# openai/robogym

Measured on AMD Instinct MI355X. Metric: env-steps/sec (whole node) dactyl/locked batch 8192; qpos L∞ vs MuJoCo (as restated by the in-repo CPU oracle: parity unpinned), higher is better.
Workload: dtype f32

## Files before the change

include/rgstep.h:

```cpp
#ifndef RGSTEP_H
#define RGSTEP_H
#include <stddef.h>
#include <stdint.h>

#ifdef __cplusplus
extern "C" {
#endif

typedef struct rg_model rg_model;
typedef struct rg_batch rg_batch;

enum {
  RG_F_QPOS = 0,
  RG_F_QVEL = 1,
  RG_F_CTRL = 2,
  RG_F_PID = 3,
  RG_F_WARMSTART = 4,
  RG_F_TIME = 5,
  RG_F_STATUS = 6,
  RG_F_STATS = 7,
  RG_F_DEBUG = 8,
  RG_F_COST = 9,
  RG_F_PAIRLB = 10,
  RG_F_ENVPRM = 11
// ... 108 lines not shown
  const float *u, *n, *e;
  const long long* action_index;
  const float* bins; int nbins;
  float* action_out;
  const float* qpos; int qpos_stride;
  const int* hand_q;
  const float* pos_to_ctrl;
  float* prm; int prm_stride;
  int p_ctrlrange, p_timestep, p_xfrc_cube, p_mass_cube;
  int relative_action, nsubsteps, fixed_wrist, wrist_act, wrist_qadr;
  float wrist_lo, wrist_hi;
  const float* obs; int obs_stride;
  const float *goal_pos, *goal_quat, *qpos_goal;
  const int* is_goal_achieved;
  const float* contact; int contact_stride, ncon_slots;
  const float* ncon; int ncon_stride;
  const float* env_reward;
  const unsigned char* env_done;
  const int* successes_so_far;
  float *out, *reward_out;
  unsigned char *done_out, *fell_out;
  int* info_out;
  float occ_geom[5]; int n_occ;
  float timestep0, cube_body_z, fall_z, occ_cutoff, ff_p, cf_p, freeze_scale, drop_reward, clip;
  int min_episode_length;
  float unc[4];
} rg_wrap_args;
int rg_wrap_layout(const rg_wrap_dims* dims, rg_wrap_lay* lay);
int rg_wrap_pre_step(const rg_wrap_args* args, void* stream);
int rg_wrap_post_step(const rg_wrap_args* args, void* stream);
int rg_wrap_args_size(void);
int rg_batch_set_constants(rg_batch* b, const int* mask_dev, void* stream);
int rg_batch_mpr_pair(rg_batch* b, int g1, int g2, float margin, float* out_dev, void* stream);
int rg_batch_items_info(const rg_batch* b, int* slots, int* queues);
int rg_obs_dim(const rg_batch* b);
int rg_debug_size(void);
int rg_lds_bytes(void);
int rg_lds_bytes_cfg(int config);
typedef struct rb_model rb_model;
typedef struct rb_batch rb_batch;
rb_model* rb_model_create(const void* blob, size_t nbytes, char* err, int errlen);
rb_model* rb_compile_mjcf(const char* xml, const char* meshdir, char* err, int errlen);
int rb_model_enable_env_params(rb_model* m);
int rb_prm_layout(const rb_model* m, int* out, int n);
int rb_model_blob_keys(const rb_model* m, char* out, int outlen);
void rb_model_free(rb_model* m);
int rb_model_info(const rb_model* m, int* out, int n);
int rb_scratch_offset(const rb_model* m, int which);
rb_batch* rb_batch_create(const rb_model* m, int B);
void rb_batch_free(rb_batch* b);
int rb_batch_reset(rb_batch* b);
int rb_batch_set_env(rb_batch* b, int hand_qposadr, int n_hand_jnt, int relative_action, const float* pos_to_ctrl);
int rb_batch_set_action_limits(rb_batch* b, float max_position_change, unsigned ctrl_centre_mask);
void* rb_batch_field_ptr(rb_batch* b, int field, int* row_words);
int rb_batch_step(rb_batch* b, const float* action_dev, const int* active_dev, int nsubsteps, int nforward_ticks, int flags, void* stream);
int rb_batch_step_ex(rb_batch* b, const float* action_dev, const int* active_dev, const int* hold_dev, const int* nticks_dev, int nsubsteps, int nforward_ticks, int flags, void* stream);
enum {
  RB_F_MOCAP = 12,
  RB_F_EQ_DATA = 13,
  RB_F_EQ_ACTIVE = 14,
  RB_F_SENSORDATA = 15
};
typedef struct rb_tcp_args {
  int arm_qposadr[6], main_arm_qposadr[6];
  int main_gripper_actuator, tcp_body, wrist_joint, reset_controller_error;
  float max_position_change, speed_roll, speed_pitch, joint_drift_threshold, gripper_ctrl_lo, gripper_ctrl_hi;
// ... 119 lines not shown
```

robogym_amd/_native.py:

```python
import ctypes
import os

import numpy as np

_HERE = os.path.dirname(os.path.abspath(__file__))
LIB_PATH = os.environ.get("RGSTEP_LIB") or os.path.join(_HERE, "csrc", "librgstep.so")

RG_F_QPOS, RG_F_QVEL, RG_F_CTRL, RG_F_PID, RG_F_WARMSTART, RG_F_TIME, RG_F_STATUS, RG_F_STATS, RG_F_DEBUG, RG_F_COST, RG_F_PAIRLB, RG_F_ENVPRM = range(12)
RB_F_MOCAP, RB_F_EQ_DATA, RB_F_EQ_ACTIVE, RB_F_SENSORDATA = 12, 13, 14, 15
RG_STATUS_BAD_STATE, RG_STATUS_CON_FULL, RG_STATUS_CAND_FULL, RG_STATUS_ROW_FULL, RG_STATUS_BAD_FACTOR, RG_STATUS_BAD_ACTION = 1, 2, 4, 8, 16, 32


class StepArgs(ctypes.Structure):

    _fields_ = [("action_dev", ctypes.c_void_p), ("goal_quat_dev", ctypes.c_void_p), ("obs_dev", ctypes.c_void_p), ("goal_dist_dev", ctypes.c_void_p),
                ("active_dev", ctypes.c_void_p), ("hold_dev", ctypes.c_void_p), ("nticks_dev", ctypes.c_void_p), ("order_dev", ctypes.c_void_p),
                ("nsubsteps", ctypes.c_int), ("nforward_ticks", ctypes.c_int), ("flags", ctypes.c_int), ("stream", ctypes.c_void_p),
                ("config", ctypes.c_int), ("redo_dev", ctypes.c_void_p), ("preticks_dev", ctypes.c_void_p), ("xdata_dev", ctypes.c_void_p)]


RG_CFG_ROLLOUT, RG_CFG_LARGE = 0, 1
RG_POST_NDRAW = 2 + 4 + 3 + 20


# ... 97 lines not shown

    _fields_ = [(n, ctypes.c_int) for n in ("nq", "nv", "nu", "nh", "ntip", "ndelta", "randomize", "relative_goal")]


class WrapLay(ctypes.Structure):

    _fields_ = ([(n, ctypes.c_int) for n in ("fwidth", "iwidth", "W", "s_prev", "s_ema", "s_alpha", "s_aema", "s_hist", "s_slack", "s_cdown", "s_cup", "s_anmult", "s_anadd", "s_addb",
                                             "s_mulb", "s_ts", "s_wind", "s_occl", "s_ffbuf", "s_ffleft", "s_cfleft", "s_cfbuf", "s_delta", "i_emat", "i_steps", "i_drops", "i_first",
                                             "i_delay", "n_action", "n_wind")]
                + [("n_noise", ctypes.c_int * 4)] + [(n, ctypes.c_int) for n in ("u_ts", "u_wind", "u_axis", "u_ff", "u_cf")] + [("key", ctypes.c_int * len(RG_WRAP_KEYS))])


def _wrap_fields():
    p_, i_, f_ = ctypes.c_void_p, ctypes.c_int, ctypes.c_float
    return ([("B", i_), ("device", i_), ("dims", WrapDims), ("lay", WrapLay), ("fstate", p_), ("istate", p_), ("u", p_), ("n", p_), ("e", p_),
             ("action_index", p_), ("bins", p_), ("nbins", i_), ("action_out", p_), ("qpos", p_), ("qpos_stride", i_), ("hand_q", p_), ("pos_to_ctrl", p_),
             ("prm", p_), ("prm_stride", i_)]
            + [(n, i_) for n in ("p_ctrlrange", "p_timestep", "p_xfrc_cube", "p_mass_cube", "relative_action", "nsubsteps", "fixed_wrist", "wrist_act", "wrist_qadr")]
            + [("wrist_lo", f_), ("wrist_hi", f_), ("obs", p_), ("obs_stride", i_), ("goal_pos", p_), ("goal_quat", p_), ("qpos_goal", p_), ("is_goal_achieved", p_),
               ("contact", p_), ("contact_stride", i_), ("ncon_slots", i_), ("ncon", p_), ("ncon_stride", i_), ("env_reward", p_), ("env_done", p_), ("successes_so_far", p_),
               ("out", p_), ("reward_out", p_), ("done_out", p_), ("fell_out", p_), ("info_out", p_), ("occ_geom", f_ * 5), ("n_occ", i_)]
            + [(n, f_) for n in ("timestep0", "cube_body_z", "fall_z", "occ_cutoff", "ff_p", "cf_p", "freeze_scale", "drop_reward", "clip")]
            + [("min_episode_length", i_), ("unc", f_ * 4)])


class WrapArgs(ctypes.Structure):

    _fields_ = _wrap_fields()


EXPORTS = [
    "rg_model_create", "rg_model_free", "rg_model_dims", "rg_batch_create", "rg_batch_free", "rg_batch_set_env",
    "rg_batch_copy", "rg_batch_reset", "rg_batch_step", "rg_obs_dim", "rg_debug_size", "rg_lds_bytes", "rg_sync",
    "rg_last_error", "rg_batch_mpr_pair", "rg_batch_copy_rows", "rg_batch_step_ex", "rg_batch_field_ptr", "rg_model_create_on", "rg_model_npair",
    "rg_lds_bytes_cfg", "rg_env_post_step", "rg_post_args_size", "rg_batch_enable_env_params", "rg_prm_layout", "rg_xdata_layout", "rg_batch_set_constants", "rg_batch_items_info",
    "rb_model_create", "rb_model_free", "rb_model_info", "rb_scratch_offset", "rb_batch_create", "rb_batch_free", "rb_batch_reset", "rb_batch_set_env",
    "rb_batch_field_ptr", "rb_batch_step", "rb_batch_step_ex", "rb_env_post_step", "rb_post_args_size", "rb_cube_ops", "rb_batch_step_tcp", "ra_env_post_step", "ra_post_args_size",
    "rg_blob_entry", "rg_model_blob_keys", "rb_model_blob_keys", "rg_compile_mjcf", "rb_compile_mjcf", "rg_compile_mjcf_blob", "rg_blob_free",
    "rb_model_enable_env_params", "rb_prm_layout", "rb_batch_set_action_limits", "ra_env_recipe_step", "ra_recipe_args_size", "rb_tcp_args_size", "rb_multi_begin", "rb_multi_launch",
    "rg_wrap_layout", "rg_wrap_pre_step", "rg_wrap_post_step", "rg_wrap_args_size",
]
EXPORTS_SETCONST = ["rb_batch_set_constants"]



class NativeError(RuntimeError):
    pass


def bind(path):
    if not os.path.exists(path):
        raise NativeError(
            "%s not found: build it with `python -c 'import __graft_entry__ as g; g.build()'` "
            "(hipcc --offload-arch=gfx950). There is no CPU fallback." % path
        )
    L = ctypes.CDLL(path)
    vp, ci, cf = ctypes.c_void_p, ctypes.c_int, ctypes.c_float
    L.rg_model_create.restype = vp
    L.rg_model_create.argtypes = [ctypes.c_char_p, ctypes.c_size_t, ctypes.c_char_p, ci]
    L.rg_model_free.argtypes = [vp]
    L.rg_model_create_on.restype = vp
    L.rg_model_create_on.argtypes = [ctypes.c_char_p, ctypes.c_size_t, ci, ctypes.c_char_p, ci]
    L.rg_model_npair.argtypes = [vp]
    L.rg_batch_step_ex.argtypes = [vp, ctypes.POINTER(StepArgs)]
    L.rg_batch_field_ptr.restype = vp
    L.rg_batch_field_ptr.argtypes = [vp, ci, ctypes.POINTER(ci)]
    L.rg_model_dims.argtypes = [vp, ctypes.POINTER(ci)]
    L.rg_batch_create.restype = vp
    L.rg_batch_create.argtypes = [vp, ci, ci]
    L.rg_batch_free.argtypes = [vp]
    L.rg_batch_set_env.argtypes = [vp, ctypes.POINTER(ci), ci, ctypes.POINTER(cf), cf]
    L.rg_batch_copy.argtypes = [vp, ci, vp, ci, ci]
    L.rg_batch_reset.argtypes = [vp]
    L.rg_batch_copy_rows.argtypes = [vp, ci, vp, vp, ci, ci, vp]
    L.rg_batch_step.argtypes = [vp, vp, vp, vp, vp, vp, ci, ci, ci, vp]
    L.rg_batch_mpr_pair.argtypes = [vp, ci, ci, cf, vp, vp]
    L.rg_obs_dim.argtypes = [vp]
    L.rg_debug_size.restype = ci
    L.rg_lds_bytes.restype = ci
    L.rg_lds_bytes_cfg.restype = ci
    L.rg_lds_bytes_cfg.argtypes = [ci]
    L.rg_batch_enable_env_params.argtypes = [vp]
    L.rg_prm_layout.argtypes = [ctypes.POINTER(ci), ci]
    L.rg_xdata_layout.argtypes = [ctypes.POINTER(ci), ci]
    L.rg_env_post_step.argtypes = [vp, ctypes.POINTER(PostArgs), vp]
    L.rg_post_args_size.restype = ci
    if L.rg_post_args_size() != ctypes.sizeof(PostArgs):
        raise NativeError("rg_post_args layout mismatch between include/rgstep.h and robogym_amd/_native.py")
    L.rg_wrap_layout.argtypes = [ctypes.POINTER(WrapDims), ctypes.POINTER(WrapLay)]
    L.rg_wrap_pre_step.argtypes = [ctypes.POINTER(WrapArgs), vp]
    L.rg_wrap_post_step.argtypes = [ctypes.POINTER(WrapArgs), vp]
    L.rg_wrap_args_size.restype = ci
    if L.rg_wrap_args_size() != ctypes.sizeof(WrapArgs):
        raise NativeError("rg_wrap_args layout mismatch between include/rgstep.h and robogym_amd/_native.py")
    L.rg_batch_set_constants.argtypes = [vp, vp, vp]
    L.rg_batch_items_info.argtypes = [vp, ctypes.POINTER(ci), ctypes.POINTER(ci)]
    L.rb_model_create.restype = vp
    L.rb_model_create.argtypes = [ctypes.c_char_p, ctypes.c_size_t, ctypes.c_char_p, ci]
    L.rb_model_free.argtypes = [vp]
    L.rb_model_info.argtypes = [vp, ctypes.POINTER(ci), ci]
    L.rg_blob_entry.argtypes = [ctypes.c_char_p, ctypes.c_size_t, ci, ctypes.c_char_p, ctypes.POINTER(ci), ctypes.POINTER(ctypes.c_uint)]
    L.rg_model_blob_keys.argtypes = [vp, ctypes.c_char_p, ci]
    L.rb_model_blob_keys.argtypes = [vp, ctypes.c_char_p, ci]
    L.rg_compile_mjcf.restype = vp
    L.rg_compile_mjcf.argtypes = [ctypes.c_char_p, ctypes.c_char_p, ctypes.c_char_p, ci]
    L.rb_compile_mjcf.restype = vp
    L.rb_compile_mjcf.argtypes = [ctypes.c_char_p, ctypes.c_char_p, ctypes.c_char_p, ci]
    L.rg_compile_mjcf_blob.argtypes = [ctypes.c_char_p, ctypes.c_char_p, ci, ctypes.POINTER(vp), ctypes.POINTER(ctypes.c_size_t), ctypes.c_char_p, ci]
    L.rg_blob_free.argtypes = [vp]
# ... 74 lines not shown
```

robogym_amd/csrc/rg_api.hip:

```cpp
#include "../../include/rgstep.h"
typedef rg_post_args RgPostArgs;
typedef rb_post_args RbPostArgs;
typedef ra_post_args RaPostArgs;
typedef ra_recipe_args RaRecipeArgs;
#define RG_NS rgs
#define RG_MAXCON 24
#define RG_CPOOL 768
#define RG_MAXCAND 128
#define RG_MAXCAND2 64
#include "rg_kernel.h"
#undef RG_NS
#undef RG_MAXCON
#undef RG_CPOOL
#undef RG_MAXCAND
#undef RG_MAXCAND2
#define RG_NS rgl
#define RG_SETCONST 1
#define RG_MAXCON 64
#define RG_CPOOL 2048
#define RG_MAXCAND 256
#define RG_MAXCAND2 128
#include "rg_kernel.h"
#undef RG_NS
#undef RG_MAXCON
// ... 730 lines not shown
  bt.redo = large ? nullptr : a->redo_dev;
  bt.preticks = a->preticks_dev;
  bt.xdata = a->xdata_dev;
  const bool items = (a->flags & 128) && !large && !(a->flags & (1 | 2 | 256)) && a->nsubsteps >= 2 && b->items_slots > 0;
  RgLaunch launch_args{b->model->aux, b->env, bt, a->nsubsteps, a->nforward_ticks, a->flags, items ? b->items_queues : 1};
  if (items) {
    const long long nitems = (long long)bt.B * a->nsubsteps;
    const int grid = (int)(nitems < b->items_slots ? nitems : b->items_slots);
    const size_t ldsi = rgi::rg_lds_launch_bytes(false);
    HIPCHK(hipMemsetAsync(bt.sched, 0, ((size_t)RG_SCHED_PROG + bt.B) * 4, (hipStream_t)a->stream));
    return launch(rgi::rg_step_items_kernel, grid, RG_WAVE, ldsi, 0, a->stream, b->model->dev_copy, launch_args);
  }
  const size_t lds = sens ? rgx::rg_lds_launch_bytes(prof) : (large ? rgl::rg_lds_launch_bytes(prof) : rgs::rg_lds_launch_bytes(prof));
  return launch(sens ? rgx::rg_step_kernel : large ? rgl::rg_step_kernel : rgs::rg_step_kernel, bt.B, RG_WAVE, lds, 0, a->stream, b->model->dev_copy, launch_args);
}
int rg_batch_step(rg_batch* b, const float* action_dev, const float* goal_quat_dev, float* obs_dev, float* goal_dist_dev,
                  const int* active_dev, int nsubsteps, int nforward_ticks, int flags, void* stream) {
  rg_step_args a;
  memset(&a, 0, sizeof a);
  a.action_dev = action_dev; a.goal_quat_dev = goal_quat_dev; a.obs_dev = obs_dev; a.goal_dist_dev = goal_dist_dev; a.active_dev = active_dev;
  a.nsubsteps = nsubsteps; a.nforward_ticks = nforward_ticks; a.flags = flags; a.stream = stream;
  return rg_batch_step_ex(b, &a);
}

int rg_batch_mpr_pair(rg_batch* b, int g1, int g2, float margin, float* out_dev, void* stream) {
  if (!b || !out_dev) return fail("null argument");
  const RgModelDev& d = b->model->dev;
  if (g1 < 0 || g2 < 0 || g1 >= d.ngeom || g2 >= d.ngeom) return fail("geom id out of range");
  DeviceGuard g(b->device);
  RgLaunch launch_args{b->model->aux, b->env, b->dev, 0, 0, 0, 1};
  return launch(rgs::rg_mpr_pair_kernel, b->dev.B, RG_WAVE, sizeof(rgs::RgLds), 0, stream, b->model->dev_copy, launch_args, g1, g2, margin, out_dev);
}

int rg_post_args_size(void) { return (int)sizeof(rg_post_args); }
int rg_env_post_step(rg_batch* b, const rg_post_args* args, void* stream) {
  if (!b || !args) return fail("null argument");
  if (!b->has_env) return fail("rg_batch_set_env must be called first");
  const rg_post_args& a = *args;
  if (!a.goal_dist || !a.obs || !a.t || !a.phase || !a.tries || !a.steps || !a.steps_since_last_goal || !a.successes_so_far || !a.goals_so_far || !a.consecutive ||
      !a.prev_dist || !a.prev_valid || !a.is_successful || !a.goal_quat || !a.qpos_goal || !a.preticks || !a.reward || !a.done || !a.goal_reset || !a.trial_success ||
      !a.sub_goal_ok || !a.env_crash || !a.resetting || !a.episode_started || !a.info_ssl || !a.nticks_next || !a.reset_mask || !a.live_mask || !a.goal_dist_before || !a.parallel_quats || !a.qpos0 || !a.zero_ctrl ||
      !a.ctrl_lo || !a.ctrl_hi) return fail("rg_env_post_step: a required array is NULL");
  const RgModelDev& d = b->model->dev;
  if (d.nu > 20) return fail("rg_env_post_step: nu exceeds RG_POST_NDRAW's action slots");
  DeviceGuard g(b->device);
  return launch(rg_post_step_kernel, b->dev.B, RG_WAVE, 0, sizeof(RgPostFlags), stream, b->dev, a, d.nq, d.nv, d.nu, d.npair);
}

int rg_wrap_args_size(void) { return (int)sizeof(rg_wrap_args); }
int rg_wrap_layout(const rg_wrap_dims* dims, rg_wrap_lay* lay) {
  if (!dims || !lay) return fail("rg_wrap_layout: null argument");
  const rg_wrap_dims& d = *dims;
  if (d.nq < 0 || d.nv < 0 || d.nu < 1 || d.nh < 0 || d.ntip < 0 || d.ndelta < 0) return fail("rg_wrap_layout: negative width");
  const int rnd = d.randomize != 0, rel = d.relative_goal != 0, nb = 4 + d.ntip + d.nh;
  rg_wrap_lay& L = *lay;
  int at = 0;
  const struct { int* off; int n; } fstate[] = {
    {&L.s_prev, d.nu}, {&L.s_ema, d.nu}, {&L.s_alpha, 1}, {&L.s_aema, d.nu}, {&L.s_hist, d.nu}, {&L.s_slack, d.nu}, {&L.s_cdown, d.nu}, {&L.s_cup, d.nu},
    {&L.s_anmult, d.nu}, {&L.s_anadd, d.nu}, {&L.s_addb, nb}, {&L.s_mulb, nb}, {&L.s_ts, 5}, {&L.s_wind, 1}, {&L.s_occl, d.ntip}, {&L.s_ffbuf, d.ntip},
    {&L.s_ffleft, 5}, {&L.s_cfleft, 1}, {&L.s_cfbuf, 17}, {&L.s_delta, d.ndelta}};
  for (const auto& f : fstate) { *f.off = at; at += f.n; }
  L.fwidth = at;
  at = 0;
  const struct { int* off; int n; } istate[] = {{&L.i_emat, 1}, {&L.i_steps, 1}, {&L.i_drops, 1}, {&L.i_first, 1}, {&L.i_delay, d.nu}};
  for (const auto& f : istate) { *f.off = at; at += f.n; }
  L.iwidth = at;
// ... 692 lines not shown
```

robogym_amd/csrc/rg_kernel.h:

```cpp
#ifndef RG_KERNEL_COMMON_H
#define RG_KERNEL_COMMON_H
#include "rg_types.h"

#ifdef RG_EMUL
#include "hip_emul.h"
#else
#include <hip/hip_runtime.h>
#endif

#ifdef RG_EMUL
typedef const RgModelDev& RgM;
#else
typedef const __attribute__((address_space(4))) RgModelDev& RgM;
#endif
#ifdef RG_FINE_PROF
#define RG_NPROF 56
#else
#define RG_NPROF 24
#endif
struct RgAux {
  const int *subtree_adr, *subtree;
  const uint32_t* dof_velmask;
};

struct RgLaunch { RgAux x; RgEnvDev env; RgBatchDev bt; int nsubsteps, nforward_ticks, flags, nqueues; };

struct RgCtx { const void* km; const void* kl; };
#ifdef RG_EMUL
#define RG_M(c) (*(const RgModelDev*)(c).km)
#define RG_L(c) (*(const RgLaunch*)(c).kl)
#define RG_S() (*(RgLds*)emul_lds())
#define RG_STAGE static inline
typedef const RgLaunch& RgLRef;
#else
extern __shared__ __attribute__((aligned(16))) unsigned char rg_lds_raw[];
#define RG_AS4 __attribute__((address_space(4)))
__device__ __forceinline__ unsigned long long rg_uniform(const void* p) {
  unsigned long long v = (unsigned long long)p;
  unsigned int lo = __builtin_amdgcn_readfirstlane((unsigned int)v), hi = __builtin_amdgcn_readfirstlane((unsigned int)(v >> 32));
  return ((unsigned long long)hi << 32) | lo;
}
#define RG_M(c) (*(const RG_AS4 RgModelDev*)rg_uniform((c).km))
#define RG_L(c) (*(const RG_AS4 RgLaunch*)rg_uniform((c).kl))
#define RG_S() (*(RgLds*)rg_lds_raw)
#define RG_STAGE __device__ __attribute__((noinline))
typedef const RG_AS4 RgLaunch& RgLRef;
#endif
#ifdef RG_EMUL
#define RG_STAGE_BIG static inline
// ... 792 lines not shown
        bool cont = false;
        if (dot(cross(p1.v, p3.v), p0.v) < 0) { p2 = p3; cont = true; }
        if (!cont && dot(cross(p3.v, p2.v), p0.v) < 0) { p1 = p3; cont = true; }
        if (cont) { dir = normalized(cross(p1.v - p0.v, p2.v - p0.v)); if (++guard > 64) state = MPR_DONE; }
        else { to_refine = true; guard = 0; }
      }
    } else {
      bool penetr = state == MPR_PENETR;
      bool reach = portal_reach_tol(p1, p2, p3, q, dir, tol);
      bool expand = false;
      if (!penetr) {
        if (dq < 0) { sep = dir; state = MPR_DONE; }
        else if (reach) state = MPR_DONE;
        else expand = true;
      } else if (reach || guard > max_iter) {
        finish = true; state = MPR_DONE;
      } else expand = true;
      if (expand) {
        expand_portal(p0, p1, p2, p3, q);
        guard++;
        if (!penetr && guard > 128) state = MPR_DONE;
        else to_refine = true;
      }
    }
    if (to_refine) {
      dir = portal_dir(p1, p2, p3);
      if (state != MPR_PENETR) { if (dot(dir, p1.v) >= 0) { state = MPR_PENETR; guard = 0; } else state = MPR_REFINE; }
    }
  }
  if (finish) { mpr_result(E.plane_depth, p0, p1, p2, p3, dir, depth, dir_out, pos); result = true; }
  return result;
}

__device__ __forceinline__ float obb_gap(const float* Ra, v3 ea, const float* Rb, v3 eb, v3 tw) {
  float R[9], AR[9];
  for (int i = 0; i < 3; i++) for (int j = 0; j < 3; j++) {
    R[3 * i + j] = Ra[i] * Rb[j] + Ra[3 + i] * Rb[3 + j] + Ra[6 + i] * Rb[6 + j];
    AR[3 * i + j] = fabsf(R[3 * i + j]) + 1e-6f;
  }
  v3 t = mulmT(Ra, tw);
  float ta[3] = {t.x, t.y, t.z}, a[3] = {ea.x, ea.y, ea.z}, b[3] = {eb.x, eb.y, eb.z};
  float gap = -1.f;
  for (int i = 0; i < 3; i++) gap = fmaxf(gap, fabsf(ta[i]) - (a[i] + b[0] * AR[3 * i] + b[1] * AR[3 * i + 1] + b[2] * AR[3 * i + 2]));
  for (int j = 0; j < 3; j++) gap = fmaxf(gap, fabsf(ta[0] * R[j] + ta[1] * R[3 + j] + ta[2] * R[6 + j]) - (a[0] * AR[j] + a[1] * AR[3 + j] + a[2] * AR[6 + j] + b[j]));
  if (gap > 0) return gap;
  for (int i = 0; i < 3; i++) for (int j = 0; j < 3; j++) {
    int i1 = (i + 1) % 3, i2 = (i + 2) % 3, j1 = (j + 1) % 3, j2 = (j + 2) % 3;
    float ra = a[i1] * AR[3 * i2 + j] + a[i2] * AR[3 * i1 + j];
    float rb = b[j1] * AR[3 * i + j2] + b[j2] * AR[3 * i + j1];
    if (fabsf(ta[i2] * R[3 * i1 + j] - ta[i1] * R[3 * i2 + j]) > ra + rb) return 0.f;
  }
  return -1.f;
}

__device__ __forceinline__ void make_frame(float* f) {
  v3 n = normalized(ld3(f));
  v3 y = (n.y < 0.5f && n.y > -0.5f) ? mk3(0, 1, 0) : mk3(0, 0, 1);
  y = normalized(y - n * dot(n, y));
  st3(f, n); st3(f + 3, y); st3(f + 6, cross(n, y));
}
__device__ __forceinline__ void add_contact(RgLds& s, int pair, float dist, v3 pos, v3 normal, int dim) {
  int c = s.ncon;
  SYNC();
  if (c >= RG_MAXCON) { if (LANE == 0) s.status |= RG_STATUS_CON_FULL; return; }
  if (LANE == 0) {
    s.c_dist[c] = dist; st3(s.c_pos + 3 * c, pos); st3(s.c_normal + 3 * c, normalized(normal));
    s.c_pair[c] = pair; s.c_dim[c] = dim; s.ncon = c + 1;
  }
  SYNC();
}

__device__ __forceinline__ MprEnv rg_mpr_env(RgM m, float* prof, bool cells) {
  MprEnv E;
  E.mesh_vert = m.mesh_vert; E.cell_adr = m.mesh_cell_adr; E.cell_blk = (const rgf4*)m.mesh_cell_blk; E.cell_ovf = (const rgf4*)m.mesh_cell_ovf;
  E.prof = prof; E.cells = cells; E.plane_depth = false;
  return E;
}
__device__ __forceinline__ void rg_mpr_geoms(RgM m, const RgLds& s, int p, float gscale, MprGeom& A, MprGeom& B, int& dim, float& margin) {
  const rgf4* R = (const rgf4*)m.pair_rec + (RG_PAIRREC / 4) * p;
  rgf4 r0 = R[0], r1 = R[1], r2 = R[2], r3 = R[3];
  int hdr = __builtin_bit_cast(int, r0.x), g1 = hdr & 255, g2 = (hdr >> 8) & 255;
  dim = (hdr >> 16) & 15; margin = r0.y;
  A.type = (hdr >> 20) & 15; A.quat = s.gquat + 4 * g1; A.size = mk3(r1.x, r1.y, r1.z); A.margin = 0.5f * margin; A.pos = mk3(0, 0, 0);
  B.type = (hdr >> 24) & 15; B.quat = s.gquat + 4 * g2; B.size = mk3(r2.x, r2.y, r2.z); B.margin = 0.5f * margin; B.pos = ld3(s.gpos + 3 * g2) - ld3(s.gpos + 3 * g1);
  if (hdr & RG_PAIR_SCALED1) A.size = A.size * gscale;
  if (hdr & RG_PAIR_SCALED2) B.size = B.size * gscale;
// ... 136 lines not shown
      if (hit) {
        int cc = cb + __popcll(bal & ((1ull << LANE) - 1ull));
        if (cc < RG_MAXCON) { s.c_dist[cc] = dist; st3(s.c_pos + 3 * cc, pos); st3(s.c_normal + 3 * cc, normalized(nrm)); s.c_pair[cc] = p; s.c_dim[cc] = dim; }
        else s.status |= RG_STATUS_CON_FULL;
      }
      if (LANE == 0) { int nn = cb + __popcll(bal); s.ncon = nn < RG_MAXCON ? nn : RG_MAXCON; }
      SYNC();
    }
  }
}
template <int G> RG_STAGE void rg_narrow_phase1(RgCtx c, int ncand) {
  RgM m = RG_M(c); RgLRef L = RG_L(c); RgLds& s = RG_S();
  bool cells = !(L.flags & 8);
  rgf4* sepdir = L.bt.sepdir ? (rgf4*)L.bt.sepdir + (size_t)rg_env(L) * m.npair : (rgf4*)0;
  float* pairlb = (L.bt.pairlb && !(L.flags & 4)) ? L.bt.pairlb + (size_t)rg_env(L) * m.npair : (float*)0;
  const float gscale = rg_prm(m, L)[RG_PRM_GEOM_SCALE];
  MprEnv E = rg_mpr_env(m, (float*)0, cells);
  const bool boxbox = !(L.flags & 16);
  for (int base = 0; base < ncand; base += RG_WAVE / G) {
    int ci = base + LANE / G;
    bool keep = false; int p = 0;
    if (ci < ncand) {
      p = s.cand[ci];
      MprGeom A, B; int dim; float margin;
      rg_mpr_geoms(m, s, p, gscale, A, B, dim, margin);
      if (A.type != RG_GEOM_PLANE && !(boxbox && A.type == RG_GEOM_BOX && B.type == RG_GEOM_BOX)) {
        v3 c0 = A.pos - B.pos;
        if (mz(c0.x) && mz(c0.y) && mz(c0.z)) c0.x += 1e-6f;
        v3 dir = normalized(c0 * -1.0f);
        if (sepdir) { rgf4 cd; const float* sp_ = (const float*)(sepdir + p); cd.x = RG_ROW_LD(sp_); cd.y = RG_ROW_LD(sp_ + 1); cd.z = RG_ROW_LD(sp_ + 2); cd.w = 0.f; if (cd.x * cd.x + cd.y * cd.y + cd.z * cd.z > 0.5f) dir = mk3(cd.x, cd.y, cd.z); }
        SupPt p1; mpr_support<G>(E, A, B, dir, p1);
        float d = dot(p1.v, dir);
        keep = d > 0;
        if (!keep && pairlb && (LANE & (G - 1)) == 0) RG_ROW_ST(pairlb + p, fmaxf(-d - 1e-6f, 0.f));
      }
    }
    bool lead = keep && (LANE & (G - 1)) == 0;
    unsigned long long bal = __ballot(lead);
    int cbase = s.ncand2;
    SYNC();
    if (lead) {
      int slot = cbase + __popcll(bal & ((1ull << LANE) - 1ull));
      if (slot < RG_MAXCAND2) s.cand2[slot] = p; else s.status |= RG_STATUS_CAND_FULL;
    }
    if (LANE == 0) { int n = cbase + __popcll(bal); s.ncand2 = n < RG_MAXCAND2 ? n : RG_MAXCAND2; }
    SYNC();
  }
}
template <int G> RG_STAGE_BIG void rg_narrow_phase2(RgCtx c, int ncand2) {
  RgM m = RG_M(c); RgLRef L = RG_L(c); RgLds& s = RG_S();
  bool cells = !(L.flags & 8);
  float* prof = (L.flags & 2) ? s.prof : (float*)0;
  rgf4* sepdir = L.bt.sepdir ? (rgf4*)L.bt.sepdir + (size_t)rg_env(L) * m.npair : (rgf4*)0;
  const float gscale = rg_prm(m, L)[RG_PRM_GEOM_SCALE];
  MprEnv E = rg_mpr_env(m, prof, cells);
  E.plane_depth = (L.flags & 16) != 0;
  for (int base = 0; base < ncand2; base += RG_WAVE / G) {
    int ci = base + LANE / G;
    bool hit = false;
    float depth = 0, margin = 0; v3 dir = mk3(0, 0, 0), pos = mk3(0, 0, 0); int p = 0, dim = 3;
    bool active = ci < ncand2;
    MprGeom A, B;
    if (active) {
      p = s.cand2[ci];
      rg_mpr_geoms(m, s, p, gscale, A, B, dim, margin);
    }
    v3 sep;
    hit = rg_mpr<G>(E, A, B, m.mpr_iterations, m.mpr_tolerance, depth, dir, pos, sep, active);
    if (active) {
      if (sepdir && (LANE & (G - 1)) == 0) { rgf4 cd; cd.x = hit ? 0.f : sep.x; cd.y = hit ? 0.f : sep.y; cd.z = hit ? 0.f : sep.z; cd.w = 0.f; RG_SEPDIR_ST(sepdir + p, cd); }
      hit = hit && dot(dir, dir) > 0.25f;
      pos = pos + ld3(s.gpos + 3 * (m.pair_gg[p] & 255));
    }
    bool lead = hit && (LANE & (G - 1)) == 0;
    unsigned long long bal = __ballot(lead);
    int cbase = s.ncon;
    SYNC();
    if (lead) {
      int c = cbase + __popcll(bal & ((1ull << LANE) - 1ull));
      if (c < RG_MAXCON) {
        s.c_dist[c] = margin - depth; st3(s.c_pos + 3 * c, pos); st3(s.c_normal + 3 * c, normalized(dir));
        s.c_pair[c] = p; s.c_dim[c] = dim;
      } else s.status |= RG_STATUS_CON_FULL;
    }
    if (LANE == 0) { int n = cbase + __popcll(bal); s.ncon = n < RG_MAXCON ? n : RG_MAXCON; }
    SYNC();
  }
}
__device__ __forceinline__ void rg_collision(RgCtx c, RgM m, RgLds& s, const float* P, float* prof, rgf4* sepdir, float* pairlb, bool cells) {
  long long tb0 = rg_clock();
  const float gscale = P[RG_PRM_GEOM_SCALE];
  if (LANE == 0) { s.ncand = 0; s.ncon = 0; }
  SYNC();
  int nround = (m.npair + RG_WAVE - 1) / RG_WAVE;
  float hb = 1.5f * P[RG_PRM_TIMESTEP];
  int nt = 0; bool bbany = false, plany = false;
  int gg_next[4]; float lb_next[4];
#pragma unroll
  for (int k = 0; k < 4; k++) { int p = k * RG_WAVE + LANE, pc = p < m.npair ? p : m.npair - 1; gg_next[k] = m.pair_gg[pc]; lb_next[k] = pairlb ? RG_ROW_LD(pairlb + pc) : 0.f; }
  for (int r0 = 0; r0 < nround; r0 += 4) {
    int gg[4]; float lbv[4];
#pragma unroll
    for (int k = 0; k < 4; k++) { gg[k] = gg_next[k]; lbv[k] = lb_next[k]; }
    if (r0 + 4 < nround) {
#pragma unroll
      for (int k = 0; k < 4; k++) { int p = (r0 + 4 + k) * RG_WAVE + LANE, pc = p < m.npair ? p : m.npair - 1; gg_next[k] = m.pair_gg[pc]; lb_next[k] = pairlb ? RG_ROW_LD(pairlb + pc) : 0.f; }
    }
#pragma unroll
    for (int k = 0; k < 4; k++) {
      int p = (r0 + k) * RG_WAVE + LANE;
      bool need = false;
      if (p < m.npair) {
        int g1 = gg[k] & 255, g2 = gg[k] >> 8;
        float lb = lbv[k] - (hb * (s.gspeed[g1] + s.gspeed[g2]) + 1e-7f);
        need = !(lb > 0.f);
        if (!need) RG_ROW_ST(pairlb + p, lb);
      }
      unsigned long long nb = __ballot(need);
      if (need) s.tlist[nt + __popcll(nb & ((1ull << LANE) - 1ull))] = (short)p;
      nt += __popcll(nb);
    }
    if (nt <= RG_TLIST - 4 * RG_WAVE && r0 + 4 < nround) continue;
    SYNC();
#ifdef RG_FINE_PROF
    const long long tref0 = rg_clock();
    if (prof && LANE == 0) { prof[42] += (float)nt; prof[43] += (float)((nt + RG_WAVE - 1) / RG_WAVE); }
#endif
    for (int i0 = 0; i0 < nt; i0 += RG_WAVE) {
      int i = i0 + LANE, q = 0;
      bool hit = false, isbb = false, ispl = false;
      if (i < nt) {
        q = s.tlist[i];
        const rgf4* R = (const rgf4*)m.pair_rec + (RG_PAIRREC / 4) * q;
        rgf4 r0 = R[0], r3 = R[3], r4 = R[4], r5 = R[5];
        int hdr = __builtin_bit_cast(int, r0.x), g1 = hdr & 255, g2 = (hdr >> 8) & 255;
        float margin = r0.y, newlb = 0.f;
        const float sc1 = (hdr & RG_PAIR_SCALED1) ? gscale : 1.f, sc2 = (hdr & RG_PAIR_SCALED2) ? gscale : 1.f;
        r3.z *= sc1; r3.w *= sc2;
        v3 p1 = ld3(s.gpos + 3 * g1), p2 = ld3(s.gpos + 3 * g2), dif = p2 - p1;
        isbb = ((hdr >> 20) & 255) == (RG_GEOM_BOX | (RG_GEOM_BOX << 4)); ispl = ((hdr >> 20) & 15) == RG_GEOM_PLANE;
        if (((hdr >> 20) & 15) == RG_GEOM_PLANE) {
          float d = dot(dif, qrot(ldq(s.gquat + 4 * g1), mk3(0, 0, 1))) - (r3.w + margin);
          hit = d <= 0; newlb = fmaxf(d, 0.f);
        } else {
          float d = sqrtf(dot(dif, dif)) - (r3.z + r3.w + margin);
          if (d <= 0) {
            float hm = 0.5f * margin + 1e-6f;
            v3 ea = mk3(r4.x * sc1 + hm, r4.y * sc1 + hm, r4.z * sc1 + hm), eb = mk3(r5.x * sc2 + hm, r5.y * sc2 + hm, r5.z * sc2 + hm);
            float Ra[9], Rb[9]; q2mat(Ra, ldq(s.gquat + 4 * g1)); q2mat(Rb, ldq(s.gquat + 4 * g2));
            float og = obb_gap(Ra, ea, Rb, eb, dif);
            hit = og < 0; newlb = fmaxf(og, 0.f);
          } else newlb = d;
        }
        if (pairlb) RG_ROW_ST(pairlb + q, fmaxf(newlb - 1e-6f, 0.f));
      }
      unsigned long long bal = __ballot(hit);
      bbany = bbany || (hit && isbb); plany = plany || (hit && ispl);
      int base = s.ncand;
      SYNC();
      if (hit) {
        int slot = base + __popcll(bal & ((1ull << LANE) - 1ull));
        if (slot < RG_MAXCAND) s.cand[slot] = q; else s.status |= RG_STATUS_CAND_FULL;
      }
      if (LANE == 0) { int n = base + __popcll(bal); s.ncand = n < RG_MAXCAND ? n : RG_MAXCAND; }
      SYNC();
    }
#ifdef RG_FINE_PROF
    if (prof && LANE == 0) prof[44] += (float)(rg_clock() - tref0);
#endif
    nt = 0;
  }
  if (prof && LANE == 0) prof[5] += (float)(rg_clock() - tb0);
  int ncand = s.ncand;
  if (LANE == 0) s.ncand2 = 0;
  SYNC();
  if (ncand > 16) rg_narrow_phase1<2>(c, ncand); else rg_narrow_phase1<4>(c, ncand);
  int ncand2 = s.ncand2;
  if (prof && LANE == 0) { prof[16] += (float)(rg_clock() - tb0); prof[17] += ncand; prof[18] += ncand2; }
  rg_narrow_phase2<4>(c, ncand2);
  if (prof && LANE == 0) prof[19] += (float)(rg_clock() - tb0);
  if (!(RG_L(c).flags & 16) && __ballot(bbany) != 0) rg_narrow_boxbox(c, ncand);
  if (__ballot(plany) != 0)
  for (int cbase = 0; cbase < ncand; cbase += RG_WAVE) {
  bool is_plane = false;
  if (cbase + LANE < ncand) is_plane = ((__builtin_bit_cast(int, m.pair_rec[RG_PAIRREC * s.cand[cbase + LANE]]) >> 20) & 15) == RG_GEOM_PLANE;
  unsigned long long plane_bits = __ballot(is_plane);
  while (plane_bits) {
    int ci = cbase + __builtin_ctzll(plane_bits); plane_bits &= plane_bits - 1;
    int p = s.cand[ci];
    int g1 = m.pair_geom[3 * p], g2 = m.pair_geom[3 * p + 1], dim = m.pair_geom[3 * p + 2];
    float margin = m.pair_prm[12 * p];
    int t2 = m.geom_type[g2];
    v3 p1 = ld3(s.gpos + 3 * g1), p2 = ld3(s.gpos + 3 * g2);
    MprGeom B;
    B.type = t2; B.quat = s.gquat + 4 * g2; B.size = ld3(m.geom_size + 3 * g2); B.margin = 0; B.mesh = -1; B.vertadr = 0; B.nvert = 0;
    if (__builtin_bit_cast(int, m.pair_rec[RG_PAIRREC * p]) & RG_PAIR_SCALED2) B.size = B.size * gscale;
    if (t2 == RG_GEOM_MESH) { B.mesh = m.geom_dataid[g2]; B.vertadr = m.mesh_vertadr[B.mesh]; B.nvert = m.mesh_vertnum[B.mesh]; }
    v3 n = qrot(ldq(s.gquat + 4 * g1), mk3(0, 0, 1));
    if (t2 == RG_GEOM_BOX) {
      int cnt = 0;
      for (int i = 0; i < 8 && cnt < 4; i++) {
        v3 lc = mk3((i & 1) ? B.size.x : -B.size.x, (i & 2) ? B.size.y : -B.size.y, (i & 4) ? B.size.z : -B.size.z);
        v3 c = qrot(ldq(B.quat), lc) + p2;
// ... 1653 lines not shown
      }
    }
  }
}
#endif

#if !RG_ITEMS
__global__ void __launch_bounds__(RG_WAVE) rg_mpr_pair_kernel(const RgModelDev* mp, RgLaunch launch, int g1, int g2, float margin, float* out) {
  RG_MAKE_CTX();
  RgM m = RG_M(c);
  RgLRef L = RG_L(c);
  RgLds& s = RG_S();
  int e = blockIdx.x;
  PFOR(i, m.nq) s.qpos[i] = L.bt.qpos[(size_t)e * m.nq + i];
  SYNC();
  st_kinematics(c);
  MprGeom A, B;
  v3 p1 = ld3(s.gpos + 3 * g1), p2 = ld3(s.gpos + 3 * g2);
  A.type = m.geom_type[g1]; A.quat = s.gquat + 4 * g1; A.size = ld3(m.geom_size + 3 * g1); A.margin = 0.5f * margin; A.pos = mk3(0, 0, 0);
  B.type = m.geom_type[g2]; B.quat = s.gquat + 4 * g2; B.size = ld3(m.geom_size + 3 * g2); B.margin = 0.5f * margin; B.pos = p2 - p1;
  A.mesh = B.mesh = -1; A.vertadr = B.vertadr = 0; A.nvert = B.nvert = 0;
  if (A.type == RG_GEOM_MESH) { A.mesh = m.geom_dataid[g1]; A.vertadr = m.mesh_vertadr[A.mesh]; A.nvert = m.mesh_vertnum[A.mesh]; }
  if (B.type == RG_GEOM_MESH) { B.mesh = m.geom_dataid[g2]; B.vertadr = m.mesh_vertadr[B.mesh]; B.nvert = m.mesh_vertnum[B.mesh]; }
  MprEnv E = rg_mpr_env(m, (float*)0, true);
  E.plane_depth = true;
  float depth = 0; v3 dir = mk3(0, 0, 0), pos = mk3(0, 0, 0);
  v3 sep; bool hit = rg_mpr<64>(E, A, B, m.mpr_iterations, m.mpr_tolerance, depth, dir, pos, sep, true);
  if (LANE == 0) {
    float* o = out + 8 * (size_t)e;
    o[0] = hit ? 1.f : 0.f; o[1] = depth; o[2] = dir.x; o[3] = dir.y; o[4] = dir.z; o[5] = pos.x + p1.x; o[6] = pos.y + p1.y; o[7] = pos.z + p1.z;
  }
}

#if RG_SETCONST
struct RgSetconstX { float cdof[6 * RG_MAXNV], off[3 * RG_MAXBODY], x[RG_MAXNV], y[RG_MAXNV], dg[RG_MAXNV]; };
static inline size_t rg_lds_setconst_bytes() { return sizeof(RgLds) + sizeof(RgSetconstX); }
__global__ void __launch_bounds__(RG_WAVE) rg_setconst_kernel(const RgModelDev* mp, RgLaunch launch, float* envprm) {
  RG_MAKE_CTX();
  RgM m = RG_M(c);
  RgLRef L = RG_L(c);
  RgLds& s = RG_S();
  RgSetconstX& X = *(RgSetconstX*)((char*)&s + sizeof(RgLds));
  const int e = blockIdx.x;
  if (e >= L.bt.B) return;
  if (L.bt.active && !L.bt.active[e]) return;
  PFOR(i, m.nq) s.qpos[i] = m.qpos0[i];
  if (LANE == 0) { s.has_xfrc = 0; s.status = 0; }
  st_build_row_desc(c);
  SYNC();
  st_kinematics(c); st_com_pos(c); st_tendon(c);
  PFOR(i, 6 * m.nv) X.cdof[i] = s.cdof[i];
  for (int b = 1 + LANE; b < m.nbody; b += RG_WAVE) st3(X.off + 3 * b, rg_xipos(m, s, b) - ld3(s.org + 3 * s.b2org[b]));
  SYNC();
  st_crb(c);
  LtdlDesc D;
  rg_ltdl_load(m.ltdl_tri, m.ltdl_pair, m.n_tri_rounds, m.n_pair_rounds, D);
  rg_M_to_blocks(m, s);
  const int d = LANE; const bool on = d < m.nv;
  const int blk = on ? m.dof_blk[d] : 0, akk = (blk & 0xFFFF) + d - ((blk >> 16) & 255);
  rg_ltdl_factor(s, D);
  float* P = envprm + (size_t)e * RG_NPRM;
  for (int i = 0; i < m.nv; i++) {
    if (on) X.x[d] = d == i ? 1.f : 0.f;
    SYNC();
    rg_ltdl_solve(s, D, X.x, d, on, akk);
    if (LANE == 0) X.dg[i] = X.x[i];
// ... 62 lines not shown
```

Baseline: 2.008 million.

## Cache separating axis in pair lower bound and prefilter with cheap axis test

The OBB gap routine now records which separating axis proved separation, including cross-product edge axes with a real normalized distance, and packs that axis index into the low 4 bits of the stored per-pair lower bound. Broadphase adds a prefilter pass that re-tests expired pairs with the bounding-sphere distance and then only the cached axis, dropping pairs still separated before the full 15-axis OBB test. This is meant to cut full OBB tests on pairs that stay apart over consecutive steps. In exchange it adds an extra compaction pass with synchronisation, slightly perturbs stored lower bounds via bit packing, and adds a standalone probe kernel for testing.

```diff
diff --git a/include/rgstep.h b/include/rgstep.h
--- a/include/rgstep.h
+++ b/include/rgstep.h
@@ -164,6 +164,7 @@
 int rg_wrap_args_size(void);
 int rg_batch_set_constants(rg_batch* b, const int* mask_dev, void* stream);
 int rg_batch_mpr_pair(rg_batch* b, int g1, int g2, float margin, float* out_dev, void* stream);
+int rg_obb_gap_probe(const float* in_dev, float* out_dev, int n, int axis, void* stream);
 int rg_batch_items_info(const rg_batch* b, int* slots, int* queues);
 int rg_obs_dim(const rg_batch* b);
 int rg_debug_size(void);
diff --git a/robogym_amd/_native.py b/robogym_amd/_native.py
--- a/robogym_amd/_native.py
+++ b/robogym_amd/_native.py
@@ -153,7 +153,7 @@
 EXPORTS = [
     "rg_model_create", "rg_model_free", "rg_model_dims", "rg_batch_create", "rg_batch_free", "rg_batch_set_env",
     "rg_batch_copy", "rg_batch_reset", "rg_batch_step", "rg_obs_dim", "rg_debug_size", "rg_lds_bytes", "rg_sync",
-    "rg_last_error", "rg_batch_mpr_pair", "rg_batch_copy_rows", "rg_batch_step_ex", "rg_batch_field_ptr", "rg_model_create_on", "rg_model_npair",
+    "rg_last_error", "rg_batch_mpr_pair", "rg_obb_gap_probe", "rg_batch_copy_rows", "rg_batch_step_ex", "rg_batch_field_ptr", "rg_model_create_on", "rg_model_npair",
     "rg_lds_bytes_cfg", "rg_env_post_step", "rg_post_args_size", "rg_batch_enable_env_params", "rg_prm_layout", "rg_xdata_layout", "rg_batch_set_constants", "rg_batch_items_info",
     "rb_model_create", "rb_model_free", "rb_model_info", "rb_scratch_offset", "rb_batch_create", "rb_batch_free", "rb_batch_reset", "rb_batch_set_env",
     "rb_batch_field_ptr", "rb_batch_step", "rb_batch_step_ex", "rb_env_post_step", "rb_post_args_size", "rb_cube_ops", "rb_batch_step_tcp", "ra_env_post_step", "ra_post_args_size",
@@ -196,6 +196,7 @@
     L.rg_batch_copy_rows.argtypes = [vp, ci, vp, vp, ci, ci, vp]
     L.rg_batch_step.argtypes = [vp, vp, vp, vp, vp, vp, ci, ci, ci, vp]
     L.rg_batch_mpr_pair.argtypes = [vp, ci, ci, cf, vp, vp]
+    L.rg_obb_gap_probe.argtypes = [vp, vp, ci, ci, vp]
     L.rg_obs_dim.argtypes = [vp]
     L.rg_debug_size.restype = ci
     L.rg_lds_bytes.restype = ci
diff --git a/robogym_amd/csrc/rg_api.hip b/robogym_amd/csrc/rg_api.hip
--- a/robogym_amd/csrc/rg_api.hip
+++ b/robogym_amd/csrc/rg_api.hip
@@ -786,6 +786,11 @@
   return launch(rgs::rg_mpr_pair_kernel, b->dev.B, RG_WAVE, sizeof(rgs::RgLds), 0, stream, b->model->dev_copy, launch_args, g1, g2, margin, out_dev);
 }
 
+int rg_obb_gap_probe(const float* in_dev, float* out_dev, int n, int axis, void* stream) {
+  if (!in_dev || !out_dev || n <= 0 || axis < 0 || axis > 15) return fail("rg_obb_gap_probe: bad argument");
+  return launch(rgs::rg_obb_gap_kernel, (n + RG_WAVE - 1) / RG_WAVE, RG_WAVE, 0, 0, stream, in_dev, out_dev, n, axis);
+}
+
 int rg_post_args_size(void) { return (int)sizeof(rg_post_args); }
 int rg_env_post_step(rg_batch* b, const rg_post_args* args, void* stream) {
   if (!b || !args) return fail("null argument");
diff --git a/robogym_amd/csrc/rg_kernel.h b/robogym_amd/csrc/rg_kernel.h
--- a/robogym_amd/csrc/rg_kernel.h
+++ b/robogym_amd/csrc/rg_kernel.h
@@ -14,7 +14,7 @@
 typedef const __attribute__((address_space(4))) RgModelDev& RgM;
 #endif
 #ifdef RG_FINE_PROF
-#define RG_NPROF 56
+#define RG_NPROF 64
 #else
 #define RG_NPROF 24
 #endif
@@ -873,7 +873,7 @@
   return result;
 }
 
-__device__ __forceinline__ float obb_gap(const float* Ra, v3 ea, const float* Rb, v3 eb, v3 tw) {
+__device__ __forceinline__ float obb_gap(const float* Ra, v3 ea, const float* Rb, v3 eb, v3 tw, int& axis) {
   float R[9], AR[9];
   for (int i = 0; i < 3; i++) for (int j = 0; j < 3; j++) {
     R[3 * i + j] = Ra[i] * Rb[j] + Ra[3 + i] * Rb[3 + j] + Ra[6 + i] * Rb[6 + j];
@@ -882,17 +882,38 @@
   v3 t = mulmT(Ra, tw);
   float ta[3] = {t.x, t.y, t.z}, a[3] = {ea.x, ea.y, ea.z}, b[3] = {eb.x, eb.y, eb.z};
   float gap = -1.f;
-  for (int i = 0; i < 3; i++) gap = fmaxf(gap, fabsf(ta[i]) - (a[i] + b[0] * AR[3 * i] + b[1] * AR[3 * i + 1] + b[2] * AR[3 * i + 2]));
-  for (int j = 0; j < 3; j++) gap = fmaxf(gap, fabsf(ta[0] * R[j] + ta[1] * R[3 + j] + ta[2] * R[6 + j]) - (a[0] * AR[j] + a[1] * AR[3 + j] + a[2] * AR[6 + j] + b[j]));
-  if (gap > 0) return gap;
+  axis = 0;
+  for (int i = 0; i < 3; i++) { float g = fabsf(ta[i]) - (a[i] + b[0] * AR[3 * i] + b[1] * AR[3 * i + 1] + b[2] * AR[3 * i + 2]); if (g > gap) { gap = g; axis = 1 + i; } }
+  for (int j = 0; j < 3; j++) { float g = fabsf(ta[0] * R[j] + ta[1] * R[3 + j] + ta[2] * R[6 + j]) - (a[0] * AR[j] + a[1] * AR[3 + j] + a[2] * AR[6 + j] + b[j]); if (g > gap) { gap = g; axis = 4 + j; } }
+  if (gap > 0) return fmaxf(gap - 2.5e-7f, 0.f);
+  axis = 0;
+  bool apart = false;
   for (int i = 0; i < 3; i++) for (int j = 0; j < 3; j++) {
     int i1 = (i + 1) % 3, i2 = (i + 2) % 3, j1 = (j + 1) % 3, j2 = (j + 2) % 3;
     float ra = a[i1] * AR[3 * i2 + j] + a[i2] * AR[3 * i1 + j];
     float rb = b[j1] * AR[3 * i + j2] + b[j2] * AR[3 * i + j1];
-    if (fabsf(ta[i2] * R[3 * i1 + j] - ta[i1] * R[3 * i2 + j]) > ra + rb) return 0.f;
-  }
-  return -1.f;
-}
+    float tl = fabsf(ta[i2] * R[3 * i1 + j] - ta[i1] * R[3 * i2 + j]);
+    if (tl > ra + rb) {
+      float l2 = R[3 * i1 + j] * R[3 * i1 + j] + R[3 * i2 + j] * R[3 * i2 + j];
+      if (l2 >= 1e-4f) { axis = 7 + 3 * i + j; return fmaxf((tl - (ra + rb) - 1e-6f) / sqrtf(l2 + 4e-6f), 0.f); }
+      apart = true;
+    }
+  }
+  return apart ? 0.f : -1.f;
+}
+__device__ __forceinline__ float obb_axis_gap(q4 qa, v3 ea, q4 qb, v3 eb, v3 tw, int axis) {
+  const int k = axis - 7, i = axis <= 3 ? axis - 1 : k / 3, j = axis <= 6 ? axis - 4 : k - 3 * (k / 3);
+  v3 ai = qrot(qa, mk3(i == 0 ? 1.f : 0.f, i == 1 ? 1.f : 0.f, i == 2 ? 1.f : 0.f)), bj = qrot(qb, mk3(j == 0 ? 1.f : 0.f, j == 1 ? 1.f : 0.f, j == 2 ? 1.f : 0.f));
+  v3 n = axis <= 3 ? ai : axis <= 6 ? bj : cross(ai, bj);
+  float l2 = dot(n, n);
+  q4 ca = qa, cb = qb; ca.x = -ca.x; ca.y = -ca.y; ca.z = -ca.z; cb.x = -cb.x; cb.y = -cb.y; cb.z = -cb.z;
+  v3 na = qrot(ca, n), nb = qrot(cb, n);
+  float r = ea.x * fabsf(na.x) + ea.y * fabsf(na.y) + ea.z * fabsf(na.z) + eb.x * fabsf(nb.x) + eb.y * fabsf(nb.y) + eb.z * fabsf(nb.z);
+  return l2 >= 1e-4f ? (fabsf(dot(tw, n)) - r - 1e-6f) / sqrtf(l2) : -1.f;
+}
+__device__ __forceinline__ float lb_pack(float lb, int axis) { return __builtin_bit_cast(float, (__builtin_bit_cast(int, lb) & ~15) | axis); }
+__device__ __forceinline__ float lb_value(float w) { return __builtin_bit_cast(float, __builtin_bit_cast(int, w) & ~15); }
+__device__ __forceinline__ int lb_axis(float w) { return __builtin_bit_cast(int, w) & 15; }
 
 __device__ __forceinline__ void make_frame(float* f) {
   v3 n = normalized(ld3(f));
@@ -1095,7 +1116,7 @@
         SupPt p1; mpr_support<G>(E, A, B, dir, p1);
         float d = dot(p1.v, dir);
         keep = d > 0;
-        if (!keep && pairlb && (LANE & (G - 1)) == 0) RG_ROW_ST(pairlb + p, fmaxf(-d - 1e-6f, 0.f));
+        if (!keep && pairlb && (LANE & (G - 1)) == 0) RG_ROW_ST(pairlb + p, lb_pack(fmaxf(-d - 1e-6f, 0.f), 0));
       }
     }
     bool lead = keep && (LANE & (G - 1)) == 0;
@@ -1157,7 +1178,8 @@
   SYNC();
   int nround = (m.npair + RG_WAVE - 1) / RG_WAVE;
   float hb = 1.5f * P[RG_PRM_TIMESTEP];
-  int nt = 0; bool bbany = false, plany = false;
+  const bool tagged = m.npair <= 2048;
+  int nt = 0, nk = 0; bool bbany = false, plany = false;
   int gg_next[4]; float lb_next[4];
 #pragma unroll
   for (int k = 0; k < 4; k++) { int p = k * RG_WAVE + LANE, pc = p < m.npair ? p : m.npair - 1; gg_next[k] = m.pair_gg[pc]; lb_next[k] = pairlb ? RG_ROW_LD(pairlb + pc) : 0.f; }
@@ -1175,49 +1197,103 @@
       bool need = false;
       if (p < m.npair) {
         int g1 = gg[k] & 255, g2 = gg[k] >> 8;
-        float lb = lbv[k] - (hb * (s.gspeed[g1] + s.gspeed[g2]) + 1e-7f);
+        float lb = lb_value(lbv[k]) - (hb * (s.gspeed[g1] + s.gspeed[g2]) + 1e-7f);
         need = !(lb > 0.f);
-        if (!need) RG_ROW_ST(pairlb + p, lb);
+        if (!need) RG_ROW_ST(pairlb + p, lb_pack(lb, lb_axis(lbv[k])));
       }
       unsigned long long nb = __ballot(need);
-      if (need) s.tlist[nt + __popcll(nb & ((1ull << LANE) - 1ull))] = (short)p;
+#ifdef RG_FINE_PROF
+      { unsigned long long zb = __ballot(need && !(lb_value(lbv[k]) > 0.f)); if (prof && LANE == 0) prof[58] += (float)__popcll(zb); }
+#endif
+      if (need) s.tlist[nt + __popcll(nb & ((1ull << LANE) - 1ull))] = (short)(tagged ? p | (lb_axis(lbv[k]) << 11) : p);
       nt += __popcll(nb);
     }
     if (nt <= RG_TLIST - 4 * RG_WAVE && r0 + 4 < nround) continue;
     SYNC();
 #ifdef RG_FINE_PROF
     const long long tref0 = rg_clock();
-    if (prof && LANE == 0) { prof[42] += (float)nt; prof[43] += (float)((nt + RG_WAVE - 1) / RG_WAVE); }
+    if (prof && LANE == 0) { prof[42] += (float)(nt - nk); prof[43] += (float)((nt - nk + RG_WAVE - 1) / RG_WAVE); }
+#endif
+    int nt2 = nk;
+    for (int i0 = nk; i0 < nt; i0 += RG_WAVE) {
+      int i = i0 + LANE, q = 0;
+      bool keep = false;
+      int cls = 0;
+      if (i < nt) {
+        const int ent = s.tlist[i];
+        q = tagged ? ent & 2047 : ent;
+        int ax = tagged ? ent >> 11 : 0;
+        const rgf4* R = (const rgf4*)m.pair_rec + (RG_PAIRREC / 4) * q;
+        rgf4 r0 = R[0], r3 = R[3], r4 = R[4], r5 = R[5];
+        int hdr = __builtin_bit_cast(int, r0.x), g1 = hdr & 255, g2 = (hdr >> 8) & 255;
+        float margin = r0.y, newlb = 0.f;
+        const float sc1 = (hdr & RG_PAIR_SCALED1) ? gscale : 1.f, sc2 = (hdr & RG_PAIR_SCALED2) ? gscale : 1.f;
+        v3 dif = ld3(s.gpos + 3 * g2) - ld3(s.gpos + 3 * g1);
+        if (((hdr >> 20) & 15) == RG_GEOM_PLANE) { newlb = dot(dif, qrot(ldq(s.gquat + 4 * g1), mk3(0, 0, 1))) - (r3.w * sc2 + margin); ax = 0; cls = 1; }
+        else {
+          newlb = sqrtf(dot(dif, dif)) - (r3.z * sc1 + r3.w * sc2 + margin); cls = 1;
+          if (newlb <= 0 && ax) {
+            float hm = 0.5f * margin + 1e-6f;
+            newlb = obb_axis_gap(ldq(s.gquat + 4 * g1), mk3(r4.x * sc1 + hm, r4.y * sc1 + hm, r4.z * sc1 + hm), ldq(s.gquat + 4 * g2), mk3(r5.x * sc2 + hm, r5.y * sc2 + hm, r5.z * sc2 + hm), dif, ax);
+            cls = 5;
+          } else ax = 0;
+        }
+        keep = !(newlb > 0);
+        if (keep) cls = 0;
+        else if (pairlb) RG_ROW_ST(pairlb + q, lb_pack(fmaxf(newlb - 1e-6f, 0.f), ax));
+      }
+      unsigned long long kb = __ballot(keep);
+#ifdef RG_FINE_PROF
+      { unsigned long long c1 = __ballot(cls == 1), c5 = __ballot(cls == 5); if (prof && LANE == 0) { prof[54] += (float)__popcll(c1); prof[59] += (float)__popcll(c5); } }
+#endif
+      SYNC();
+      if (keep) s.tlist[nt2 + __popcll(kb & ((1ull << LANE) - 1ull))] = (short)q;
+      nt2 += __popcll(kb);
+    }
+    SYNC();
+    nt = nk = nt2;
+#ifdef RG_FINE_PROF
+    if (prof && LANE == 0) prof[44] += (float)(rg_clock() - tref0);
+#endif
+    if (nk < RG_WAVE && r0 + 4 < nround) continue;
+#ifdef RG_FINE_PROF
+    const long long tref1 = rg_clock();
+    if (prof && LANE == 0) prof[60] += (float)((nt + RG_WAVE - 1) / RG_WAVE);
 #endif
     for (int i0 = 0; i0 < nt; i0 += RG_WAVE) {
       int i = i0 + LANE, q = 0;
       bool hit = false, isbb = false, ispl = false;
+      int cls = 0;
       if (i < nt) {
         q = s.tlist[i];
         const rgf4* R = (const rgf4*)m.pair_rec + (RG_PAIRREC / 4) * q;
         rgf4 r0 = R[0], r3 = R[3], r4 = R[4], r5 = R[5];
         int hdr = __builtin_bit_cast(int, r0.x), g1 = hdr & 255, g2 = (hdr >> 8) & 255;
         float margin = r0.y, newlb = 0.f;
+        int ax = 0;
         const float sc1 = (hdr & RG_PAIR_SCALED1) ? gscale : 1.f, sc2 = (hdr & RG_PAIR_SCALED2) ? gscale : 1.f;
         r3.z *= sc1; r3.w *= sc2;
         v3 p1 = ld3(s.gpos + 3 * g1), p2 = ld3(s.gpos + 3 * g2), dif = p2 - p1;
         isbb = ((hdr >> 20) & 255) == (RG_GEOM_BOX | (RG_GEOM_BOX << 4)); ispl = ((hdr >> 20) & 15) == RG_GEOM_PLANE;
         if (((hdr >> 20) & 15) == RG_GEOM_PLANE) {
           float d = dot(dif, qrot(ldq(s.gquat + 4 * g1), mk3(0, 0, 1))) - (r3.w + margin);
-          hit = d <= 0; newlb = fmaxf(d, 0.f);
+          hit = d <= 0; newlb = fmaxf(d, 0.f); cls = hit ? 4 : 1;
         } else {
           float d = sqrtf(dot(dif, dif)) - (r3.z + r3.w + margin);
           if (d <= 0) {
             float hm = 0.5f * margin + 1e-6f;
             v3 ea = mk3(r4.x * sc1 + hm, r4.y * sc1 + hm, r4.z * sc1 + hm), eb = mk3(r5.x * sc2 + hm, r5.y * sc2 + hm, r5.z * sc2 + hm);
             float Ra[9], Rb[9]; q2mat(Ra, ldq(s.gquat + 4 * g1)); q2mat(Rb, ldq(s.gquat + 4 * g2));
-            float og = obb_gap(Ra, ea, Rb, eb, dif);
-            hit = og < 0; newlb = fmaxf(og, 0.f);
-          } else newlb = d;
+            float og = obb_gap(Ra, ea, Rb, eb, dif, ax);
+            hit = og < 0; newlb = fmaxf(og, 0.f); cls = hit ? 4 : og > 0.f ? 2 : 3;
+          } else { newlb = d; cls = 1; }
         }
-        if (pairlb) RG_ROW_ST(pairlb + q, fmaxf(newlb - 1e-6f, 0.f));
+        if (pairlb) RG_ROW_ST(pairlb + q, lb_pack(fmaxf(newlb - 1e-6f, 0.f), ax));
       }
       unsigned long long bal = __ballot(hit);
+#ifdef RG_FINE_PROF
+      for (int k = 2; k <= 4; k++) { unsigned long long cb = __ballot(cls == k); if (prof && LANE == 0) prof[53 + k] += (float)__popcll(cb); }
+#endif
       bbany = bbany || (hit && isbb); plany = plany || (hit && ispl);
       int base = s.ncand;
       SYNC();
@@ -1229,9 +1305,9 @@
       SYNC();
     }
 #ifdef RG_FINE_PROF
-    if (prof && LANE == 0) prof[44] += (float)(rg_clock() - tref0);
-#endif
-    nt = 0;
+    if (prof && LANE == 0) prof[44] += (float)(rg_clock() - tref1);
+#endif
+    nt = nk = 0;
   }
   if (prof && LANE == 0) prof[5] += (float)(rg_clock() - tb0);
   int ncand = s.ncand;
@@ -2951,6 +3027,21 @@
   }
 }
 
+__global__ void rg_obb_gap_kernel(const float* in, float* out, int n, int axis) {
+  const int k = blockIdx.x * blockDim.x + threadIdx.x;
+  if (k >= n) return;
+  const float* v = in + 17 * (size_t)k;
+  q4 qa = ldq(v), qb = ldq(v + 7);
+  v3 ea = ld3(v + 4), eb = ld3(v + 11), t = ld3(v + 14);
+  float Ra[9], Rb[9]; q2mat(Ra, qa); q2mat(Rb, qb);
+  int ax = 0;
+  float* o = out + 4 * (size_t)k;
+  o[0] = obb_gap(Ra, ea, Rb, eb, t, ax);
+  o[1] = (float)ax;
+  o[2] = ax ? obb_axis_gap(qa, ea, qb, eb, t, ax) : 0.f;
+  o[3] = axis ? obb_axis_gap(qa, ea, qb, eb, t, axis) : 0.f;
+}
+
 #if RG_SETCONST
 struct RgSetconstX { float cdof[6 * RG_MAXNV], off[3 * RG_MAXBODY], x[RG_MAXNV], y[RG_MAXNV], dg[RG_MAXNV]; };
 static inline size_t rg_lds_setconst_bytes() { return sizeof(RgLds) + sizeof(RgSetconstX); }
```

After: 1.984 million. -1.2%, worse.
